# lawmurray/BayesLogit

Measured on NVIDIA B200. Metric: pg_draws_per_sec, higher is better.
Workload: dtype f64

## Files before the change

### bayeslogit_b200/csrc/pg_alt.cuh

```cuda
#pragma once

namespace bl {

template <class Src>
__device__ __forceinline__ double alt_rtinvchi2(Src &s, double h, double trunc)
{
    double h2 = h * h;
    double R = trunc / h2;
    double E1 = s.expon();
    double E2 = s.expon();
    while ((E1 * E1) > (2 * E2 / R)) {
        E1 = s.expon();
        E2 = s.expon();
    }
    double X = 1 + E1 * R;
    X = R / (X * X);
    return h2 * X;
}

__device__ __forceinline__ double alt_pigauss(double x, double z, double lambda)
{
    double sq = sqrt(lambda / x);
    double b = sq * (x * z - 1);
    double a = sq * (x * z + 1) * -1.0;
    return p_norm(b) + ool::exp_(2 * lambda * z) * p_norm(a);
}

enum AltField {
    kAltH = 0,
    kAltTrunc,
    kAltPr,
    kAltCoef,
    kAltLgh,
    kAltLd0, kAltLd1,
    kAltLtB, kAltLtC0, kAltLtLM,
    kAltPrBand,
    kAltSetupDoubles
};
constexpr int kAltStateDoubles = 2 * kAltSetupDoubles;

struct AltState {
    double f[kAltStateDoubles];
    __device__ __forceinline__ double get(int k) const { return f[k]; }
};

struct AltStateRef {
    const double *o;
    size_t stride;
    __device__ __forceinline__ double get(int k) const { return o[(size_t)k * stride]; }
};

__device__ __forceinline__ void alt_plan(double h, int &nfull, int &nrem, double &hrem)
{
    double n = floor((h - 1.0) / 4.0);
    double remain = h - 4.0 * n;
    nfull = (int)n;
    if (remain > 4.0) {
        nrem = 2;
        hrem = 0.5 * remain;
    } else {
        nrem = 1;
        hrem = remain;
    }
}

static __device__ __noinline__ double alt_pr_fp64(double h, double z, double trunc)
{
    const double kLog2 = 0.693147180559945309417232;
    double wl, wr;
    if (z != 0)
        wl = ool::exp_(h * (kLog2 - z)) * alt_pigauss(trunc, z / h, h * h);
    else
        wl = ool::exp_(h * kLog2) * (1.0 - p_gamma_rate(1 / trunc, 0.5, 0.5 * h * h));
    double lambda_z = kPi * kPi * 0.125 + 0.5 * z * z;
    wr = ool::exp_(h * ool::log_((0.5 * kPi) / lambda_z)) * (1.0 - p_gamma_rate(trunc, h, lambda_z));
    return wr / (wr + wl);
}

constexpr double kAltPrBandWidth = 2e-5;

__device__ __forceinline__ float alt_pr_estimate(double h, double z, double trunc)
{
    const float hf = (float)h, zf = (float)z, tf = (float)trunc;
    if (!(zf < 12.0f)) return -1.0f;
    const float s = hf * rsqrtf(tf);
    const float tz = tf * zf / hf;
    const float b = s * (tz - 1.0f), na = s * (tz + 1.0f);
    const float phib = 0.5f * erfcf(-b * 0.70710678f);
    const float wl = exp2f(hf) * (__expf(-hf * zf) * phib
                                  + 0.5f * erfcxf(na * 0.70710678f) * __expf(hf * zf - 0.5f * na * na));
    const float lam = 1.2337005501361697f + 0.5f * zf * zf;
    const float x = tf * lam;
    const float lpre = hf * __logf(x) - x;
    float Q;
    if (x < hf + 1.0f) {
        float term = 1.0f, sum = 1.0f, ap = hf;
        for (int k = 0; k < 60; ++k) {
            ap += 1.0f;
            term *= x / ap;
            sum += term;
            if (term < 1e-8f * sum) break;
        }
        Q = 1.0f - sum * __expf(lpre - lgammaf(hf + 1.0f));
    } else {
        float cf = upper_gamma_cf_f32(hf, x);
        if (!(cf > 0.0f)) return -1.0f;
        Q = cf * __expf(lpre - lgammaf(hf));
    }
    if (!(Q > 0.0f)) return -1.0f;
    const float wr = __expf(hf * __logf(1.5707963267948966f / lam)) * Q;
    const float pr = wr / (wr + wl);
    return pr >= 0.0f && pr <= 1.0f ? pr : -1.0f;
}

template <bool kEstimatePr>
static __device__ __noinline__ void alt_setup(double h, double z, double *out)
{
    const double kLog2 = 0.693147180559945309417232;
    int idx = (int)floor((h - 1.0) * 100.0);
    double trunc = PG_TRUNC_SCHEDULE[idx];
    double rate_z = 0.125 * kPi * kPi + 0.5 * z * z;
    float est = kEstimatePr ? alt_pr_estimate(h, z, trunc) : -1.0f;
    out[kAltH] = h;
    out[kAltTrunc] = trunc;
    out[kAltPr] = est >= 0.0f ? (double)est : alt_pr_fp64(h, z, trunc);
    out[kAltPrBand] = est >= 0.0f ? kAltPrBandWidth : 0.0;
    out[kAltCoef] = ool::exp_(h * kLog2 - 0.5 * 1.8378770664093454835606594728112 );
    out[kAltLgh] = ool::lgamma_(h);
    out[kAltLd0] = ool::log_(h);
    out[kAltLd1] = ool::log_(2.0 + h);
    double b = rate_z * trunc;
    double d1 = b - h;
    double d3 = h - 1.0;
    double c0 = 0.5 * (d1 + sqrt(d1 * d1 + 4.0 * b)) / b;
    out[kAltLtB] = b;
    out[kAltLtC0] = c0;
    out[kAltLtLM] = d3 * ool::log_(d3 / (1.0 - c0)) - d3;
}

template <class St>
__device__ __forceinline__ bool alt_pick_right(double u, const St &st, int o, double z)
{
    const double pr = st.get(o + kAltPr), band = st.get(o + kAltPrBand);
    if (u < pr - band) return true;
    if (u > pr + band || band == 0.0) return false;
    return u < alt_pr_fp64(st.get(o + kAltH), z, st.get(o + kAltTrunc));
}

struct AltLane {
    double X, alpha, sum;
    int trial;
    int phase;
    int nfull;
    int nrem;
    __device__ __forceinline__ void start(int nf, int nr)
    {
        X = 0.0; alpha = 0.0; sum = 0.0; trial = 0; phase = 0; nfull = nf; nrem = nr;
    }
};

__device__ __forceinline__ double alt_coef(double n, double lx3, double ldn, double x, double h,
                                           double coef_h, double &g)
{
    double d_n = 2.0 * n + h;
    if (n != 0)
        g *= (n + h - 1) / n;
    else
        g = 1.0;
    double coef = coef_h * g;
    double log_kernel = -0.5 * (lx3 + d_n * d_n / x) + ldn;
    return coef * ool::exp_(log_kernel);
}

template <class Src, class St>
__device__ __forceinline__ bool alt_pick(Src &src, AltLane &L, double z, const St &st)
{
    const int o = L.nfull > 0 ? 0 : kAltSetupDoubles;
    if (L.trial >= 10000) {
        L.sum += -1.0;
        L.trial = 0;
        if (L.nfull > 0)
            L.nfull--;
        else
            L.nrem--;
        return L.nfull == 0 && L.nrem == 0;
    }
    L.trial++;
    if (alt_pick_right(src.unif(), st, o, z)) {
        L.phase = 1;
    } else {
        L.phase = (st.get(o + kAltH) / z > st.get(o + kAltTrunc)) ? 2 : 3;
        L.alpha = 0.0;
    }
    return false;
}

template <class St>
static __device__ __noinline__ bool alt_series_exact(double X, double u, double h, double trunc, const St &st, int o)
{
    const int max_inner = 200;
    const double coef_h = st.get(o + kAltCoef);
    const double lx3 = ool::log_(X * X * X);
    double g = 1.0;
    double S = alt_coef(0.0, lx3, st.get(o + kAltLd0), X, h, coef_h, g);
    double a_n = S;
    double gt;
    if (X > trunc)
        gt = ool::exp_(h * 0.45158270528945486472619522989488  + (h - 1) * (lx3 * (1.0 / 3.0))
                       - kPi * kPi * 0.125 * X - st.get(o + kAltLgh));
    else
        gt = h * ool::exp_(h * 0.693147180559945309417232 - 0.5 * (1.8378770664093454835606594728112 + lx3)
                           - 0.5 * h * h / X);
    double Y = u * gt;
    int n = 0;
    bool go = true, accept = false;
    while (go && n < max_inner) {
        ++n;
        double prev = a_n;
        double ldn = n == 1 ? st.get(o + kAltLd1) : ool::log_(2.0 * n + h);
        a_n = alt_coef((double)n, lx3, ldn, X, h, coef_h, g);
        bool decreasing = a_n <= prev;
        if (n & 1) {
            S = S - a_n;
            if (Y <= S && decreasing) {
                accept = true;
                go = false;
            }
        } else {
            S = S + a_n;
            if (Y > S && decreasing) go = false;
        }
    }
    return accept;
}

template <class St>
__device__ __forceinline__ bool alt_series_test(double X, double u, double h, double trunc, const St &st, int o)
{
    const double coef_h = st.get(o + kAltCoef);
    const double iX = 1.0 / X;
    const double lx3 = 3.0 * (double)__logf((float)X);
    double lgt;
    if (X > trunc)
        lgt = h * 0.45158270528945486472619522989488 + (h - 1) * (lx3 * (1.0 / 3.0)) - kPi * kPi * 0.125 * X
            - st.get(o + kAltLgh);
    else
        lgt = st.get(o + kAltLd0) + h * 0.693147180559945309417232 - 0.5 * (1.8378770664093454835606594728112 + lx3)
            - 0.5 * h * h * iX;
    const double base = -0.5 * lx3 - lgt;
    const double d0 = h, d1 = h + 2.0, d2 = h + 4.0;
    const double r0 = coef_h * d0 * (double)__expf((float)(base - 0.5 * d0 * d0 * iX));
    const double r1 = coef_h * h * d1 * (double)__expf((float)(base - 0.5 * d1 * d1 * iX));
    const double r2 = coef_h * (0.5 * h * (h + 1.0)) * d2 * (double)__expf((float)(base - 0.5 * d2 * d2 * iX));
    const double band = 1e-5 * (r0 + r1 + r2) + 1e-9;
    const double s1 = r0 - r1;
    if (u <= s1 - band && r1 <= r0 - band) return true;
    const bool not_at_1 = u > s1 + band || r1 > r0 + band;
    if (not_at_1 && u > s1 + r2 + band && r2 <= r1 - band) return false;
    return alt_series_exact(X, u, h, trunc, st, o);
}

template <bool kPickInside = true, class Src, class St>
__device__ __forceinline__ bool alt_trip(Src &src, AltLane &L, double z, const St &st)
{
    if (kPickInside && L.phase == 0) {
        if (alt_pick(src, L, z, st)) return true;
        if (L.phase == 0) return false;
    }
    const int o = L.nfull > 0 ? 0 : kAltSetupDoubles;
    const double h = st.get(o + kAltH);
    const double trunc = st.get(o + kAltTrunc);
    bool chunk_done = false;
    double chunk_val = 0.0;
    if (L.phase == 1) {
        double rate_z = 0.125 * kPi * kPi + 0.5 * z * z;
        if (h == 1.0) {
            L.X = src.expon() / rate_z + trunc;
            L.phase = 4;
        } else {
            double b = st.get(o + kAltLtB), c0 = st.get(o + kAltLtC0);
            double x = b + src.expon() / c0;
            double u = src.unif();
            double l_rho = (h - 1.0) * ool::log_(x) - x * (1.0 - c0);
            if (ool::log_(u) <= l_rho - st.get(o + kAltLtLM)) {
                L.X = trunc * (x / b);
                L.phase = 4;
            }
        }
    } else if (L.phase == 2) {
        if (src.unif() > L.alpha) {
            L.X = alt_rtinvchi2(src, h, trunc);
            L.alpha = ool::exp_(-0.5 * z * z * L.X);
        } else {
            L.phase = 4;
        }
    } else if (L.phase == 3) {
        double X = igauss(src, h / z, h * h);
        if (!(X > trunc)) {
            L.X = X;
            L.phase = 4;
        }
    }
    if (L.phase == 4) {
        const double X = L.X;
        const bool accept = alt_series_test(X, src.unif(), h, trunc, st, o);
        L.phase = 0;
        if (accept) {
            chunk_done = true;
            chunk_val = 0.25 * X;
        }
    }
    if (chunk_done) {
        L.sum += chunk_val;
        L.trial = 0;
        if (L.nfull > 0)
            L.nfull--;
        else
            L.nrem--;
        if (L.nfull == 0 && L.nrem == 0) return true;
    }
    return false;
}

template <class Src>
__device__ double alt_draw(Src &s, double h, double z)
{
    if (h < 1) return 0;
    if (h != h) return h;
    int nfull, nrem;
    double hrem;
    alt_plan(h, nfull, nrem, hrem);
    double zh = fabs(z) * 0.5;
    AltState st;
    if (nfull > 0) alt_setup<false>(4.0, zh, st.f);
    alt_setup<false>(hrem, zh, st.f + kAltSetupDoubles);
    AltLane L;
    L.start(nfull, nrem);
    while (!alt_trip(s, L, zh, st)) {}
    return L.sum;
}

}
```

### bayeslogit_b200/csrc/pg_hybrid.cu

```cuda
#include <algorithm>
#include <cstdlib>
#include <vector>

#include "engine.h"
#include "pg_devroye_fast.cuh"
#include "pg_stream.cuh"

namespace bl {

namespace {

constexpr int kBinThreads = 256;
constexpr int kMetaCounts = 0;
constexpr int kMetaOffsets = 8;
constexpr int kMetaCursor = 16;

__global__ void __launch_bounds__(kBinThreads)
k_hyb_count(const double *__restrict__ h, int n, int *__restrict__ meta)
{
    __shared__ int cnt[8];
    if (threadIdx.x < 8) cnt[threadIdx.x] = 0;
    __syncthreads();
    int local[6] = {0, 0, 0, 0, 0, 0};
    for (int i = blockIdx.x * blockDim.x + threadIdx.x; i < n; i += gridDim.x * blockDim.x)
        local[regime_of(h[i])]++;
#pragma unroll
    for (int r = 0; r < 6; ++r) {
        int v = local[r];
        for (int o = 16; o; o >>= 1) v += __shfl_xor_sync(0xffffffffu, v, o);
        if ((threadIdx.x & 31) == 0 && v) atomicAdd(&cnt[r], v);
    }
    __syncthreads();
    if (threadIdx.x < 6 && cnt[threadIdx.x]) atomicAdd(&meta[kMetaCounts + threadIdx.x], cnt[threadIdx.x]);
}

__global__ void k_hyb_offsets(int *meta)
{
    int acc = 0;
    for (int r = 1; r < 6; ++r) {
        meta[kMetaOffsets + r] = acc;
        meta[kMetaCursor + r] = 0;
        acc += meta[kMetaCounts + r];
    }
}

constexpr int kBinPer = 4;

__global__ void __launch_bounds__(kBinThreads)
k_hyb_scatter(const double *__restrict__ h, int n, int *__restrict__ meta, int *__restrict__ idx,
              double *__restrict__ x)
{
    constexpr int kCells = kBinPer * (kBinThreads / 32);
    __shared__ int wcnt[kCells][8];
    __shared__ int base[8];
    const int lane = threadIdx.x & 31, warp = threadIdx.x >> 5;
    const unsigned lt = (1u << lane) - 1u;
    const int tile_obs = kBinThreads * kBinPer;
    int tiles = (n + tile_obs - 1) / tile_obs;
    for (int tile = blockIdx.x; tile < tiles; tile += gridDim.x) {
        int reg[kBinPer], rank[kBinPer];
#pragma unroll
        for (int k = 0; k < kBinPer; ++k) {
            int i = tile * tile_obs + k * kBinThreads + threadIdx.x;
            reg[k] = i < n ? regime_of(h[i]) : -1;
        }
#pragma unroll
        for (int k = 0; k < kBinPer; ++k) {
            int i = tile * tile_obs + k * kBinThreads + threadIdx.x;
            if (reg[k] == kRegZero) x[i] = 0.0;
            rank[k] = 0;
#pragma unroll
            for (int r = 1; r < 6; ++r) {
                unsigned m = __ballot_sync(0xffffffffu, reg[k] == r);
                if (reg[k] == r) rank[k] = __popc(m & lt);
                if (lane == 0) wcnt[k * (kBinThreads / 32) + warp][r] = __popc(m);
            }
        }
        __syncthreads();
        if (threadIdx.x >= 1 && threadIdx.x < 6) {
            int r = threadIdx.x, run = 0;
            for (int c = 0; c < kCells; ++c) {
                int v = wcnt[c][r];
                wcnt[c][r] = run;
                run += v;
            }
            base[r] = run ? meta[kMetaOffsets + r] + atomicAdd(&meta[kMetaCursor + r], run) : 0;
        }
        __syncthreads();
#pragma unroll
        for (int k = 0; k < kBinPer; ++k) {
            if (reg[k] > 0) {
                int i = tile * tile_obs + k * kBinThreads + threadIdx.x;
                idx[base[reg[k]] + wcnt[k * (kBinThreads / 32) + warp][reg[k]] + rank[k]] = i;
            }
        }
        __syncthreads();
    }
}

template <int R, bool kChains = false>
__global__ void __launch_bounds__(128)
k_hyb_regime(double *__restrict__ x, const double *__restrict__ h, const double *__restrict__ z,
             const int *__restrict__ idx, const int *__restrict__ meta, StreamId id)
{
    const int count = meta[kMetaCounts + R];
    const int *list = idx + meta[kMetaOffsets + R];
    for (int j = blockIdx.x * blockDim.x + threadIdx.x; j < count; j += gridDim.x * blockDim.x) {
        int i = list[j];
        PhiloxSource s;
        if (kChains) open_batch_stream(s, id, i);
        else s.open(id.seed, id.obs0 + (uint64_t)i, id.call_id);
        double b = h[i], zi = z[i], v;
        if (R == kRegNormal) {
            double m = pg_m1(b, zi);
            double var = pg_m2(b, zi) - m * m;
            v = m + sqrt(var) * s.norm();
        } else if (R == kRegSP) {
            sp_draw(s, v, b, zi);
        } else if (R == kRegDevroye) {
            v = devroye_sum_fast(s, (int)b, zi);
        } else if (R == kRegAlt) {
            v = alt_draw(s, b, zi);
        } else {
            v = gamma_sum(s, b, zi, 200);
        }
        x[i] = v;
    }
}

__global__ void __launch_bounds__(128, 8)
k_sp_setup(const double *__restrict__ h, const double *__restrict__ z, const int *__restrict__ idx,
           const int *__restrict__ meta, double *__restrict__ state, int c0, int cap)
{
    const int count = min(meta[kMetaCounts + kRegSP] - c0, cap);
    const int *list = idx + meta[kMetaOffsets + kRegSP] + c0;
    for (int j = blockIdx.x * blockDim.x + threadIdx.x; j < count; j += gridDim.x * blockDim.x) {
        int i = list[j];
        SpState s;
        sp_setup<true>(h[i], z[i], s);
#pragma unroll
        for (int k = 0; k < kSpStateDoubles; ++k) state[(size_t)k * cap + j] = s.f[k];
    }
}

constexpr int kLaneChunk = 128;

constexpr int kRgThreads = 256;

template <int F, int D, int I>
struct RgSlots {
    double f[F][kRgThreads];
    double d[D][kRgThreads];
    uint4 buf[kRgThreads];
    uint32_t blk[kRgThreads];
    int pos[kRgThreads];
    int i[I][kRgThreads];
    int obs[kRgThreads];
    int phase[kRgThreads];
    int perm[kRgThreads];
    int wcnt[kRgThreads / 32][3];
};

struct SpRegroup {
    static constexpr int F = kSpStateDoubles, D = 3, I = 1, kClasses = 2, kRegime = kRegSP;
    using Slots = RgSlots<F, D, I>;
    __device__ static void begin(Slots &S, int t, double shape, double zraw, PhiloxSource &src)
    {
        S.d[0][t] = shape;
        S.d[1][t] = 0.5 * fabs(zraw);
        S.d[2][t] = 2.0;
        S.i[0][t] = 1;
        SpStateRef st{&S.f[0][t], (size_t)kRgThreads};
        S.phase[t] = sp_pick_left(src.unif(), st, shape) ? 1 : 2;
    }
    __device__ static bool advance(Slots &S, int sl, PhiloxSource &src, double &omega)
    {
        SpLane L;
        L.X = S.d[2][sl];
        L.iter = S.i[0][sl];
        L.phase = S.phase[sl];
        const double n = S.d[0][sl];
        SpStateRef st{&S.f[0][sl], (size_t)kRgThreads};
        bool done = sp_trip_staged(src, L, n, S.d[1][sl], st);
        if (!done && L.phase == 0) {
            if (L.iter >= 200) {
                done = true;
            } else {
                L.iter++;
                L.phase = sp_pick_left(src.unif(), st, n) ? 1 : 2;
            }
        }
        if (done) {
            omega = n * 0.25 * L.X;
        } else {
            S.d[2][sl] = L.X;
            S.i[0][sl] = L.iter;
            S.phase[sl] = L.phase;
        }
        return done;
    }
};

struct AltRegroup {
    static constexpr int F = kAltStateDoubles, D = 4, I = 3, kClasses = 3, kRegime = kRegAlt;
    using Slots = RgSlots<F, D, I>;
    __device__ static void load(const Slots &S, int sl, AltLane &L)
    {
        L.X = S.d[1][sl]; L.alpha = S.d[2][sl]; L.sum = S.d[3][sl];
        L.trial = S.i[0][sl]; L.nfull = S.i[1][sl]; L.nrem = S.i[2][sl];
        L.phase = S.phase[sl];
    }
    __device__ static void store(Slots &S, int sl, const AltLane &L)
    {
        S.d[1][sl] = L.X; S.d[2][sl] = L.alpha; S.d[3][sl] = L.sum;
        S.i[0][sl] = L.trial; S.i[1][sl] = L.nfull; S.i[2][sl] = L.nrem;
        S.phase[sl] = L.phase;
    }
    __device__ static void begin(Slots &S, int t, double shape, double zraw, PhiloxSource &src)
    {
        int nfull, nrem;
        double hrem;
        alt_plan(shape, nfull, nrem, hrem);
        AltLane L;
        L.start(nfull, nrem);
        const double zh = 0.5 * fabs(zraw);
        S.d[0][t] = zh;
        AltStateRef st{&S.f[0][t], (size_t)kRgThreads};
        alt_pick(src, L, zh, st);
        store(S, t, L);
    }
    __device__ static bool advance(Slots &S, int sl, PhiloxSource &src, double &omega)
    {
        AltLane L;
        load(S, sl, L);
        const double zh = S.d[0][sl];
        AltStateRef st{&S.f[0][sl], (size_t)kRgThreads};
        bool done = alt_trip<false>(src, L, zh, st);
        while (!done && L.phase == 0) done = alt_pick(src, L, zh, st);
        if (done)
            omega = L.sum;
        else
            store(S, sl, L);
        return done;
    }
};

template <class R, bool kChains = false>
__global__ void __launch_bounds__(kRgThreads)
k_loop_regroup(double *__restrict__ x, const double *__restrict__ h, const double *__restrict__ z,
               const int *__restrict__ idx, const int *__restrict__ meta, const double *__restrict__ state,
               int c0, int cap, StreamId id)
{
    using Slots = typename R::Slots;
    extern __shared__ __align__(16) unsigned char rg_raw[];
    Slots &S = *reinterpret_cast<Slots *>(rg_raw);
    const int count = min(meta[kMetaCounts + R::kRegime] - c0, cap);
    if (count <= 0) return;
    const int *list = idx + meta[kMetaOffsets + R::kRegime] + c0;
    const unsigned full = 0xffffffffu;
    const int t = threadIdx.x, lane = t & 31, warp = t >> 5;
    const unsigned lt_mask = (1u << lane) - 1u;
    constexpr int kWarps = kRgThreads / 32;
    const int gwarp = blockIdx.x * kWarps + warp;
    const int stride = gridDim.x * kWarps * kLaneChunk;
    int cur = gwarp * kLaneChunk, cend = cur + kLaneChunk;

    S.phase[t] = -1;
    __syncthreads();
    for (;;) {
        const bool empty = S.phase[t] < 0;
        const unsigned want = __ballot_sync(full, empty);
        if (want && cur < count) {
            int rank = __popc(want & lt_mask);
            int cand = cur + rank;
            if (cand >= cend) cand += stride - kLaneChunk;
            if (empty && cand < count) {
                const int obs = list[cand];
#pragma unroll
                for (int k = 0; k < R::F; ++k) S.f[k][t] = __ldg(state + (size_t)k * cap + cand);
                S.obs[t] = obs;
                PhiloxSource src;
                if (kChains) open_batch_stream(src, id, obs);
                else src.open(id.seed, id.obs0 + (uint64_t)obs, id.call_id);
                R::begin(S, t, h[obs], z[obs], src);
                S.buf[t] = src.buf;
                S.blk[t] = src.blk;
                S.pos[t] = src.pos;
            }
            cur += __popc(want);
            if (cur >= cend) {
                int over = cur - cend;
                cend += stride;
                cur = cend - kLaneChunk + over;
            }
        }
        const int ph = S.phase[t];
        const unsigned m1 = __ballot_sync(full, ph == 1), m2 = __ballot_sync(full, ph == 2);
        const unsigned m3 = R::kClasses > 2 ? __ballot_sync(full, ph == 3) : 0u;
        if (lane == 0) { S.wcnt[warp][0] = __popc(m1); S.wcnt[warp][1] = __popc(m2); S.wcnt[warp][2] = __popc(m3); }
        __syncthreads();
        int tot1 = 0, tot2 = 0, tot3 = 0, b1 = 0, b2 = 0, b3 = 0;
#pragma unroll
        for (int w = 0; w < kWarps; ++w) {
            int a = S.wcnt[w][0], b = S.wcnt[w][1], c = S.wcnt[w][2];
            if (w < warp) { b1 += a; b2 += b; b3 += c; }
            tot1 += a;
            tot2 += b;
            tot3 += c;
        }
        if (tot1 + tot2 + tot3 == 0) {
            if (!__syncthreads_or(cur < count)) break;
            continue;
        }
        if (ph == 1) S.perm[b1 + __popc(m1 & lt_mask)] = t;
        else if (ph == 3) S.perm[tot1 + b3 + __popc(m3 & lt_mask)] = t;
        else if (ph == 2) S.perm[kRgThreads - 1 - (b2 + __popc(m2 & lt_mask))] = t;
        __syncthreads();
        if (t < tot1 + tot3 || t >= kRgThreads - tot2) {
            const int sl = S.perm[t];
            PhiloxSource src;
            if (kChains) open_batch_stream(src, id, S.obs[sl]);
            else src.open(id.seed, id.obs0 + (uint64_t)S.obs[sl], id.call_id);
            src.buf = S.buf[sl];
            src.blk = S.blk[sl];
            src.pos = S.pos[sl];
            double omega;
            if (R::advance(S, sl, src, omega)) {
                x[S.obs[sl]] = omega;
                S.phase[sl] = -1;
            } else {
                S.buf[sl] = src.buf;
                S.blk[sl] = src.blk;
                S.pos[sl] = src.pos;
            }
        }
        __syncthreads();
    }
}

template <class R, bool kChains>
int regroup_grid()
{
    using Slots = typename R::Slots;
    cudaFuncSetAttribute(k_loop_regroup<R, kChains>, cudaFuncAttributeMaxDynamicSharedMemorySize, (int)sizeof(Slots));
    int per_sm = 0;
    if (cudaOccupancyMaxActiveBlocksPerMultiprocessor(&per_sm, k_loop_regroup<R, kChains>, kRgThreads, sizeof(Slots)) != cudaSuccess || per_sm < 1)
        per_sm = 1;
    int sms = 148, dev = 0;
    if (cudaGetDevice(&dev) == cudaSuccess) cudaDeviceGetAttribute(&sms, cudaDevAttrMultiProcessorCount, dev);
    return sms * per_sm;
}

__global__ void __launch_bounds__(128)
k_alt_setup(const double *__restrict__ h, const double *__restrict__ z, const int *__restrict__ idx,
            const int *__restrict__ meta, double *__restrict__ state, int c0, int cap)
{
    const int count = min(meta[kMetaCounts + kRegAlt] - c0, cap);
    const int *list = idx + meta[kMetaOffsets + kRegAlt] + c0;
    for (int j = blockIdx.x * blockDim.x + threadIdx.x; j < count; j += gridDim.x * blockDim.x) {
        int i = list[j];
        int nfull, nrem;
        double hrem, zh = 0.5 * fabs(z[i]);
        alt_plan(h[i], nfull, nrem, hrem);
        double f[kAltSetupDoubles];
        alt_setup<true>(hrem, zh, f);
#pragma unroll
        for (int k = 0; k < kAltSetupDoubles; ++k) state[(size_t)(kAltSetupDoubles + k) * cap + j] = f[k];
        if (nfull > 0) {
            alt_setup<true>(4.0, zh, f);
#pragma unroll
            for (int k = 0; k < kAltSetupDoubles; ++k) state[(size_t)k * cap + j] = f[k];
        }
    }
}

constexpr int kStateChunk = 1 << 23;
constexpr int kStateDoubles = kSpStateDoubles > kAltStateDoubles ? kSpStateDoubles : kAltStateDoubles;

template <class K>
int resident_grid(K kernel, int threads, int need)
{
    int per_sm = 0;
    if (cudaOccupancyMaxActiveBlocksPerMultiprocessor(&per_sm, kernel, threads, 0) != cudaSuccess || per_sm < 1)
        per_sm = 1;
    int sms = 148;
    int dev = 0;
    if (cudaGetDevice(&dev) == cudaSuccess) cudaDeviceGetAttribute(&sms, cudaDevAttrMultiProcessorCount, dev);
    int cap = sms * per_sm;
    return need < cap ? (need > 0 ? need : 1) : cap;
}

template <int R, bool kChains>
void launch_regime(double *x, const double *h, const double *z, const int *idx, const int *meta,
                   StreamId id, int n, cudaStream_t st)
{
    static const int cap = resident_grid(k_hyb_regime<R, kChains>, 128, 1 << 30);
    int need = (n + 127) / 128;
    k_hyb_regime<R, kChains><<<need < cap ? need : cap, 128, 0, st>>>(x, h, z, idx, meta, id);
    count_launch();
}

}

enum HybStage { kStBin = 0, kStSpSetup, kStSpLoop, kStAltSetup, kStAltLoop, kStGamma, kStNormal, kStDevroye, kStCount };
static bool g_hyb_timing = false;
static std::vector<cudaEvent_t> g_hyb_pool;
struct HybSpan { int stage; int a, b; };
static std::vector<HybSpan> g_hyb_spans;
static int g_hyb_used = 0;

void hybrid_timing_enable(bool on) { g_hyb_timing = on; }

static int hyb_mark(cudaStream_t st)
{
    if ((int)g_hyb_pool.size() <= g_hyb_used) {
        cudaEvent_t e;
        cudaEventCreate(&e);
        g_hyb_pool.push_back(e);
    }
    cudaEventRecord(g_hyb_pool[g_hyb_used], st);
    return g_hyb_used++;
}

struct HybTimer {
    bool on;
    cudaStream_t st;
    int stage, a;
    HybTimer(bool on_, cudaStream_t st_, int stage_) : on(on_), st(st_), stage(stage_), a(on_ ? hyb_mark(st_) : 0) {}
    ~HybTimer() { if (on) g_hyb_spans.push_back(HybSpan{stage, a, hyb_mark(st)}); }
};

int hybrid_timing_last(double *ms8, int *launches8)
{
    if (g_hyb_spans.empty()) return 1;
    for (int k = 0; k < kStCount; ++k) { ms8[k] = 0.0; if (launches8) launches8[k] = 0; }
    if (cudaEventSynchronize(g_hyb_pool[g_hyb_used - 1]) != cudaSuccess) return 1;
    for (const HybSpan &sp : g_hyb_spans) {
        float ms = 0.f;
        cudaEventElapsedTime(&ms, g_hyb_pool[sp.a], g_hyb_pool[sp.b]);
        ms8[sp.stage] += ms;
        if (launches8 && ms > 0.02f) launches8[sp.stage]++;
    }
    return 0;
}

static size_t hybrid_state_offset(int64_t num) { return ((32 + (size_t)num) * sizeof(int) + 15) / 16 * 16; }

size_t hybrid_workspace_bytes(int64_t num)
{
    size_t cap = (size_t)(num < kStateChunk ? num : kStateChunk);
    return hybrid_state_offset(num) + cap * kStateDoubles * sizeof(double);
}

struct SideStream {
    cudaStream_t s = nullptr;
    cudaEvent_t fork = nullptr, join = nullptr;
    cudaStream_t get()
    {
        if (!s) {
            int lo = 0, hi = 0;
            cudaDeviceGetStreamPriorityRange(&lo, &hi);
            cudaStreamCreateWithPriority(&s, cudaStreamNonBlocking, lo);
            cudaEventCreateWithFlags(&fork, cudaEventDisableTiming);
            cudaEventCreateWithFlags(&join, cudaEventDisableTiming);
        }
        return s;
    }
};
static SideStream g_side;

template <bool kChains>
static cudaError_t launch_hybrid_binned_k(double *x, const double *h, const double *z, int num, StreamId id,
                                          void *work, cudaStream_t st)
{
    if (num <= 0) return cudaSuccess;
    int *meta = (int *)work;
    int *idx = meta + 32;
    cudaError_t e = cudaMemsetAsync(meta, 0, 32 * sizeof(int), st);
    if (e != cudaSuccess) return e;
    int tiles = (num + kBinThreads - 1) / kBinThreads;
    int grid = tiles < 148 * 8 ? tiles : 148 * 8;
    int stiles = (num + kBinThreads * kBinPer - 1) / (kBinThreads * kBinPer);
    int sgrid = stiles < 148 * 8 ? stiles : 148 * 8;
    const bool tm = g_hyb_timing;
    if (tm) { g_hyb_spans.clear(); g_hyb_used = 0; }
    {
        HybTimer t(tm, st, kStBin);
        k_hyb_count<<<grid, kBinThreads, 0, st>>>(h, num, meta);
        k_hyb_offsets<<<1, 1, 0, st>>>(meta);
        k_hyb_scatter<<<sgrid, kBinThreads, 0, st>>>(h, num, meta, idx, x);
        count_launch(3);
    }
    static const bool use_side = getenv("BL_HYBRID_NO_SIDE_STREAM") == nullptr;
    cudaStream_t side = use_side ? g_side.get() : st;
    if (use_side) {
        cudaEventRecord(g_side.fork, st);
        cudaStreamWaitEvent(side, g_side.fork, 0);
    }
    {
        HybTimer t(tm, side, kStGamma);
        launch_regime<kRegGamma, kChains>(x, h, z, idx, meta, id, num, side);
    }
    {
        HybTimer t(tm, side, kStNormal);
        launch_regime<kRegNormal, kChains>(x, h, z, idx, meta, id, num, side);
    }
    {
        HybTimer t(tm, side, kStDevroye);
        launch_regime<kRegDevroye, kChains>(x, h, z, idx, meta, id, num, side);
    }
    double *state = (double *)((char *)work + hybrid_state_offset(num));
    const int cap = num < kStateChunk ? num : kStateChunk;
    static const int g_sp_setup = resident_grid(k_sp_setup, 128, 1 << 30);
    static const int g_alt_setup = resident_grid(k_alt_setup, 128, 1 << 30);
    static const int g_sp_regroup = regroup_grid<SpRegroup, kChains>();
    static const int g_alt_regroup = regroup_grid<AltRegroup, kChains>();
    const int rneed = (cap + kLaneChunk * (kRgThreads / 32) - 1) / (kLaneChunk * (kRgThreads / 32));
    const int sneed = (cap + 127) / 128;
    for (int c0 = 0; c0 < num; c0 += cap) {
        {
            HybTimer t(tm, st, kStSpSetup);
            k_sp_setup<<<std::min(sneed, g_sp_setup), 128, 0, st>>>(h, z, idx, meta, state, c0, cap);
        }
        {
            HybTimer t(tm, st, kStSpLoop);
            k_loop_regroup<SpRegroup, kChains><<<std::min(rneed, g_sp_regroup), kRgThreads, sizeof(SpRegroup::Slots), st>>>(x, h, z, idx, meta, state, c0, cap, id);
        }
        count_launch(2);
    }
    for (int c0 = 0; c0 < num; c0 += cap) {
        {
            HybTimer t(tm, st, kStAltSetup);
            k_alt_setup<<<std::min(sneed, g_alt_setup), 128, 0, st>>>(h, z, idx, meta, state, c0, cap);
        }
        {
            HybTimer t(tm, st, kStAltLoop);
            k_loop_regroup<AltRegroup, kChains><<<std::min(rneed, g_alt_regroup), kRgThreads, sizeof(AltRegroup::Slots), st>>>(x, h, z, idx, meta, state, c0, cap, id);
        }
        count_launch(2);
    }
    if (use_side) {
        cudaEventRecord(g_side.join, side);
        cudaStreamWaitEvent(st, g_side.join, 0);
    }
    return cudaGetLastError();
}

cudaError_t launch_hybrid_binned(double *x, const double *h, const double *z, int num, StreamId id,
                                 void *work, cudaStream_t st)
{
    return id.chain_len ? launch_hybrid_binned_k<true>(x, h, z, num, id, work, st)
                        : launch_hybrid_binned_k<false>(x, h, z, num, id, work, st);
}

}
```

### bayeslogit_b200/csrc/pg_samplers.cuh

```cuda
#pragma once

#include "philox.cuh"
#include "specfun.cuh"

#define PG_TABLE_QUAL static __device__ __constant__
#include "pg_tables.h"

namespace bl {

constexpr double kTrunc = 0.64;

namespace ool {
static __device__ __noinline__ double log_(double x) { return ::log(x); }
static __device__ __noinline__ double exp_(double x) { return ::exp(x); }
static __device__ __noinline__ double tan_(double x) { return ::tan(x); }
static __device__ __noinline__ double tanh_(double x) { return ::tanh(x); }
static __device__ __noinline__ double cos_(double x) { return ::cos(x); }
static __device__ __noinline__ double cosh_(double x) { return ::cosh(x); }
static __device__ __noinline__ double atan_(double x) { return ::atan(x); }
static __device__ __noinline__ double lgamma_(double x) { return ::lgamma(x); }
static __device__ __noinline__ double tgamma_(double x) { return ::tgamma(x); }
}


__device__ __forceinline__ double dev_coef(int n, double x)
{
    double K = (n + 0.5) * kPi;
    if (x > kTrunc) return K * exp(-0.5 * K * K * x);
    if (x > 0) {
        double e = -1.5 * (log(0.5 * kPi) + log(x)) + log(K) - 2.0 * (n + 0.5) * (n + 0.5) / x;
        return exp(e);
    }
    return 0.0;
}

__device__ __forceinline__ double dev_right_mass(double Z)
{
    const double t = kTrunc;
    double fz = 0.125 * kPi * kPi + 0.5 * Z * Z;
    double b = sqrt(1.0 / t) * (t * Z - 1);
    double a = sqrt(1.0 / t) * (t * Z + 1) * -1.0;
    double x0 = log(fz) + fz * t;
    double xb = x0 - Z + log_p_norm(b);
    double xa = x0 + Z + log_p_norm(a);
    double qdivp = 4 / kPi * (exp(xb) + exp(xa));
    return 1.0 / (1.0 + qdivp);
}

__device__ __forceinline__ double dev_fz(double Z)
{
    return __dadd_rn(0.125 * kPi * kPi, __dmul_rn(__dmul_rn(0.5, Z), Z));
}

__device__ __forceinline__ double dev_x_right(double E, double fz)
{
    return __dadd_rn(kTrunc, __ddiv_rn(E, fz));
}

__device__ __forceinline__ double dev_x_pair(double E1)
{
    double X = __dadd_rn(1.0, __dmul_rn(E1, kTrunc));
    return __ddiv_rn(kTrunc, __dmul_rn(X, X));
}

__device__ __forceinline__ double dev_x_ig(double N, double mu)
{
    double Y = __dmul_rn(N, N);
    double half_mu = __dmul_rn(0.5, mu);
    double mu_Y = __dmul_rn(mu, Y);
    double rad = __dsqrt_rn(__dadd_rn(__dmul_rn(4.0, mu_Y), __dmul_rn(mu_Y, mu_Y)));
    return __dadd_rn(__dadd_rn(mu, __dmul_rn(half_mu, mu_Y)), -__dmul_rn(half_mu, rad));
}

__device__ __forceinline__ double dev_ig_flip_threshold(double X, double mu)
{
    return __ddiv_rn(mu, __dadd_rn(mu, X));
}

__device__ __forceinline__ double dev_x_ig_flip(double X, double mu)
{
    return __ddiv_rn(__dmul_rn(mu, mu), X);
}

template <class Src>
__device__ __forceinline__ double dev_trunc_igauss(Src &s, double Z)
{
    const double t = kTrunc;
    double X = t + 1.0;
    if (1.0 / kTrunc > Z) {
        double alpha = 0.0;
        while (s.unif() > alpha) {
            double E1 = s.expon();
            double E2 = s.expon();
            while (E1 * E1 > 2 * E2 / t) {
                E1 = s.expon();
                E2 = s.expon();
            }
            X = dev_x_pair(E1);
            alpha = exp(-0.5 * Z * Z * X);
        }
    } else {
        double mu = 1.0 / Z;
        while (X > t) {
            X = dev_x_ig(s.norm(), mu);
            if (s.unif() > dev_ig_flip_threshold(X, mu)) X = dev_x_ig_flip(X, mu);
        }
    }
    return X;
}

template <class Src>
__device__ __forceinline__ double devroye_one(Src &s, double Z, double fz, double right_mass)
{
    for (;;) {
        double X;
        if (s.unif() < right_mass)
            X = dev_x_right(s.expon(), fz);
        else
            X = dev_trunc_igauss(s, Z);
        double S = dev_coef(0, X);
        double Y = s.unif() * S;
        int n = 0;
        for (;;) {
            ++n;
            if (n & 1) {
                S = S - dev_coef(n, X);
                if (Y <= S) return 0.25 * X;
            } else {
                S = S + dev_coef(n, X);
                if (Y > S) break;
            }
        }
    }
}

template <class Src>
__device__ __forceinline__ double devroye_sum(Src &s, int n, double z)
{
    if (n < 1) n = 1;
    double Z = fabs(z) * 0.5;
    double fz = dev_fz(Z);
    double pr = dev_right_mass(Z);
    double sum = 0.0;
    for (int i = 0; i < n; ++i) sum += devroye_one(s, Z, fz, pr);
    return sum;
}


template <class Src>
__device__ __forceinline__ double gamma_sum(Src &s, double b, double z, int T)
{
    if (T < 1) T = 1;
    double x = 0.0;
    double kappa = z * z;
    for (int k = 0; k < T; ++k) {
        double d = (double)k + 0.5;
        double bk = (4 * kPi * kPi) * d * d;
        x += s.gamma(b) / (bk + kappa);
    }
    return 2.0 * x;
}


__device__ __forceinline__ double jj_m1(double b, double z)
{
    z = fabs(z);
    if (z > 1e-12) return b * tanh(z) / z;
    return b * (1 - (1.0 / 3) * pow(z, 2) + (2.0 / 15) * pow(z, 4) - (17.0 / 315) * pow(z, 6));
}

__device__ __forceinline__ double jj_m2(double b, double z)
{
    z = fabs(z);
    if (z > 1e-12) {
        double tz = tanh(z) / z;
        return (b + 1) * b * (tz * tz) + b * ((tanh(z) - z) / (z * z * z));
    }
    double p = 1 - (1.0 / 3) * pow(z, 2) + (2.0 / 15) * pow(z, 4) - (17.0 / 315) * pow(z, 6);
    return (b + 1) * b * (p * p) + b * ((-1.0 / 3) + (2.0 / 15) * pow(z, 2) - (17.0 / 315) * pow(z, 4));
}

__device__ __forceinline__ double pg_m1(double b, double z) { return jj_m1(b, 0.5 * z) * 0.25; }
__device__ __forceinline__ double pg_m2(double b, double z) { return jj_m2(b, 0.5 * z) * 0.0625; }


template <class Src>
__device__ __forceinline__ double igauss(Src &s, double mu, double lambda)
{
    double nu = s.norm();
    double y = nu * nu;
    double x = mu + 0.5 * mu * mu * y / lambda
             - 0.5 * mu / lambda * sqrt(4.0 * mu * lambda * y + (mu * y) * (mu * y));
    if (s.unif() > mu / (mu + x)) x = mu * mu / x;
    return x;
}

template <class Src>
__device__ __noinline__ double ltgamma(Src &s, double shape, double rate, double trunc)
{
    double a = shape;
    double b = rate * trunc;
    if (trunc <= 0.0 || shape < 1.0) return 0.0;
    if (shape == 1.0) return s.expon() / rate + trunc;
    double d1 = b - a;
    double d3 = a - 1.0;
    double c0 = 0.5 * (d1 + sqrt(d1 * d1 + 4.0 * b)) / b;
    double l_M = d3 * ool::log_(d3 / (1.0 - c0)) - d3;
    double x;
    for (;;) {
        x = b + s.expon() / c0;
        double u = s.unif();
        double l_rho = d3 * ool::log_(x) - x * (1.0 - c0);
        if (ool::log_(u) <= l_rho - l_M) break;
    }
    return trunc * (x / b);
}

template <class Src>
__device__ __forceinline__ double tnorm_left(Src &s, double left)
{
    if (left < 0.0) {
        for (;;) {
            double z = s.norm();
            if (z > left) return z;
        }
    }
    double astar = 0.5 * (left + sqrt(left * left + 4.0));
    for (;;) {
        double z = s.expon() / astar + left;
        double rho = ool::exp_(-0.5 * (z - astar) * (z - astar));
        if (s.unif() < rho) return z;
    }
}

template <class Src>
__device__ __forceinline__ double rtinvchi2(Src &s, double scale, double trunc)
{
    double R = trunc / scale;
    double z = tnorm_left(s, 1.0 / sqrt(R));
    return scale / (z * z);
}

}

#include "pg_alt.cuh"
#include "pg_sp.cuh"

namespace bl {


enum Regime { kRegZero = 0, kRegGamma = 1, kRegDevroye = 2, kRegAlt = 3, kRegSP = 4, kRegNormal = 5 };

__device__ __forceinline__ int regime_of(double b)
{
    if (b > 170) return kRegNormal;
    if (b > 13) return kRegSP;
    if (b == 1 || b == 2) return kRegDevroye;
    if (b > 1) return kRegAlt;
    if (b > 0) return kRegGamma;
    return kRegZero;
}

template <class Src>
__device__ double devroye_sum_fast(Src &s, int n, double z);

template <class Src>
__device__ double hybrid_draw(Src &s, double b, double z, int &aux)
{
    aux = 0;
    switch (regime_of(b)) {
    case kRegNormal: {
        double m = pg_m1(b, z);
        double v = pg_m2(b, z) - m * m;
        return m + sqrt(v) * s.norm();
    }
    case kRegSP: {
        double d;
        aux = sp_draw(s, d, b, z);
        return d;
    }
    case kRegDevroye:
        return devroye_sum_fast(s, (int)b, z);
    case kRegAlt:
        return alt_draw(s, b, z);
    case kRegGamma:
        return gamma_sum(s, b, z, 200);
    default:
        return 0.0;
    }
}

}
```

Baseline: 5.080 billion.

## Run alt-regime trips to completion with float-guarded accept tests and deeper series bounds

Adds a staged trip for the alternate PG sampler. Each proposal phase now runs until it produces a candidate and goes straight to the series test, so the per-lane X and alpha no longer need to be stored in the regroup slots. The truncated inverse-chi2 and thinning loops and the left-truncated gamma accept step use lazy exponentials and float logs, with an error band that falls back to exact double evaluation only near the boundary. The series test now evaluates five terms instead of three before falling back to the exact series. The aim is less slot traffic, fewer double-precision transcendentals and fewer exact-series calls, in exchange for more divergence inside the warp and more code complexity.

```diff
diff --git a/bayeslogit_b200/csrc/pg_alt.cuh b/bayeslogit_b200/csrc/pg_alt.cuh
--- a/bayeslogit_b200/csrc/pg_alt.cuh
+++ b/bayeslogit_b200/csrc/pg_alt.cuh
@@ -1,6 +1,13 @@
 #pragma once
 
 namespace bl {
+
+__device__ __forceinline__ double alt_invchi2_x(double E1, double h2, double R)
+{
+    double X = 1 + E1 * R;
+    X = R / (X * X);
+    return h2 * X;
+}
 
 template <class Src>
 __device__ __forceinline__ double alt_rtinvchi2(Src &s, double h, double trunc)
@@ -13,9 +20,7 @@
         E1 = s.expon();
         E2 = s.expon();
     }
-    double X = 1 + E1 * R;
-    X = R / (X * X);
-    return h2 * X;
+    return alt_invchi2_x(E1, h2, R);
 }
 
 __device__ __forceinline__ double alt_pigauss(double x, double z, double lambda)
@@ -248,30 +253,51 @@
         lgt = st.get(o + kAltLd0) + h * 0.693147180559945309417232 - 0.5 * (1.8378770664093454835606594728112 + lx3)
             - 0.5 * h * h * iX;
     const double base = -0.5 * lx3 - lgt;
-    const double d0 = h, d1 = h + 2.0, d2 = h + 4.0;
-    const double r0 = coef_h * d0 * (double)__expf((float)(base - 0.5 * d0 * d0 * iX));
-    const double r1 = coef_h * h * d1 * (double)__expf((float)(base - 0.5 * d1 * d1 * iX));
-    const double r2 = coef_h * (0.5 * h * (h + 1.0)) * d2 * (double)__expf((float)(base - 0.5 * d2 * d2 * iX));
-    const double band = 1e-5 * (r0 + r1 + r2) + 1e-9;
-    const double s1 = r0 - r1;
-    if (u <= s1 - band && r1 <= r0 - band) return true;
-    const bool not_at_1 = u > s1 + band || r1 > r0 + band;
-    if (not_at_1 && u > s1 + r2 + band && r2 <= r1 - band) return false;
+    auto rn = [&](double g, double d) { return coef_h * g * d * (double)__expf((float)(base - 0.5 * d * d * iX)); };
+    const double g2 = 0.5 * h * (h + 1.0), g3 = g2 * (h + 2.0) * (1.0 / 3.0);
+    const double r0 = rn(1.0, h), r1 = rn(h, h + 2.0), r2 = rn(g2, h + 4.0), r3 = rn(g3, h + 6.0),
+                 r4 = rn(g3 * (h + 3.0) * 0.25, h + 8.0);
+    const double band = 1e-5 * (r0 + r1 + r2 + r3 + r4) + 1e-9;
+    auto step = [&](bool odd, double S, double r, double p) {
+        if ((odd ? u <= S - band : u > S + band) && r <= p - band) return 1;
+        return (odd ? u > S + band : u <= S - band) || r > p + band ? 0 : -1;
+    };
+    const double s1 = r0 - r1, s2 = s1 + r2, s3 = s2 - r3;
+    int k = step(true, s1, r1, r0);
+    if (k == 1) return true;
+    if (k == 0) {
+        k = step(false, s2, r2, r1);
+        if (k == 1) return false;
+        if (k == 0) {
+            k = step(true, s3, r3, r2);
+            if (k == 1) return true;
+            if (k == 0 && step(false, s3 + r4, r4, r3) == 1) return false;
+        }
+    }
     return alt_series_exact(X, u, h, trunc, st, o);
 }
 
-template <bool kPickInside = true, class Src, class St>
+__device__ __forceinline__ bool alt_chunk_done(AltLane &L, double X)
+{
+    L.sum += 0.25 * X;
+    L.trial = 0;
+    if (L.nfull > 0)
+        L.nfull--;
+    else
+        L.nrem--;
+    return L.nfull == 0 && L.nrem == 0;
+}
+
+template <class Src, class St>
 __device__ __forceinline__ bool alt_trip(Src &src, AltLane &L, double z, const St &st)
 {
-    if (kPickInside && L.phase == 0) {
+    if (L.phase == 0) {
         if (alt_pick(src, L, z, st)) return true;
         if (L.phase == 0) return false;
     }
     const int o = L.nfull > 0 ? 0 : kAltSetupDoubles;
     const double h = st.get(o + kAltH);
     const double trunc = st.get(o + kAltTrunc);
-    bool chunk_done = false;
-    double chunk_val = 0.0;
     if (L.phase == 1) {
         double rate_z = 0.125 * kPi * kPi + 0.5 * z * z;
         if (h == 1.0) {
@@ -305,21 +331,87 @@
         const double X = L.X;
         const bool accept = alt_series_test(X, src.unif(), h, trunc, st, o);
         L.phase = 0;
-        if (accept) {
-            chunk_done = true;
-            chunk_val = 0.25 * X;
-        }
-    }
-    if (chunk_done) {
-        L.sum += chunk_val;
-        L.trial = 0;
-        if (L.nfull > 0)
-            L.nfull--;
-        else
-            L.nrem--;
-        if (L.nfull == 0 && L.nrem == 0) return true;
+        if (accept) return alt_chunk_done(L, X);
     }
     return false;
+}
+
+static __device__ __noinline__ bool alt_pair_again_exact(uint32_t w1, int k1, uint32_t w2, int k2, double R)
+{
+    const double E1 = philox_expon_ool(w1, k1), E2 = philox_expon_ool(w2, k2);
+    return (E1 * E1) > (2 * E2 / R);
+}
+
+static __device__ __noinline__ bool alt_thin_again_exact(double u, double a)
+{
+    return u > ool::exp_(a);
+}
+
+template <class St>
+__device__ __forceinline__ bool alt_trip_staged(PhiloxSource &src, AltLane &L, double z, const St &st)
+{
+    const int o = L.nfull > 0 ? 0 : kAltSetupDoubles;
+    const double h = st.get(o + kAltH);
+    const double trunc = st.get(o + kAltTrunc);
+    double X;
+    if (L.phase == 1) {
+        if (h == 1.0) {
+            double rate_z = 0.125 * kPi * kPi + 0.5 * z * z;
+            X = src.expon() / rate_z + trunc;
+        } else {
+            const double b = st.get(o + kAltLtB), c0 = st.get(o + kAltLtC0), l_M = st.get(o + kAltLtLM);
+            const double x = b + src.expon() / c0;
+            const double u = src.unif();
+            const float lx = __logf((float)x), lu = __logf((float)u);
+            const double d = (h - 1.0) * (double)lx - x * (1.0 - c0) - l_M - (double)lu;
+            const double band = 1.25e-6 * ((h - 1.0) * (1.0 + fabs((double)lx)) + 2.0 + fabs((double)lu));
+            bool ok;
+            if (!(fabs(d) < 700.0)) ok = sp_ltgamma_accept_exact(u, x, h, c0, l_M);
+            else if (d > band) ok = true;
+            else if (d < -band) ok = false;
+            else ok = sp_ltgamma_accept_exact(u, x, h, c0, l_M);
+            if (!ok) return false;
+            X = trunc * (x / b);
+        }
+    } else if (L.phase == 2) {
+        const double h2 = h * h;
+        const double R = trunc / h2;
+        const double hz2 = -0.5 * z * z;
+        src.word();
+        for (;;) {
+            PhiloxSource::LazyE l1, l2;
+            for (;;) {
+                l1 = src.expon_lazy();
+                l2 = src.expon_lazy();
+                const double e1 = (double)PhiloxSource::approx(l1), e2 = (double)PhiloxSource::approx(l2);
+                const double d = 0.5 * R * (e1 * e1) - e2;
+                const double band = 1.25e-6 * (1.0 + e2 + R * e1 * (1.0 + e1));
+                bool again;
+                if (d > band) again = true;
+                else if (d < -band) again = false;
+                else again = alt_pair_again_exact(l1.w, l1.k, l2.w, l2.k, R);
+                if (!again) break;
+            }
+            X = alt_invchi2_x(philox_expon_ool(l1.w, l1.k), h2, R);
+            const double a = hz2 * X;
+            const double u = src.unif();
+            const float lu = __logf((float)u);
+            const double d = (double)lu - a;
+            const double band = 1.25e-6 * (1.0 + fabs((double)lu));
+            bool again;
+            if (!(a > -700.0)) again = alt_thin_again_exact(u, a);
+            else if (d > band) again = true;
+            else if (d < -band) again = false;
+            else again = alt_thin_again_exact(u, a);
+            if (!again) break;
+        }
+    } else {
+        X = igauss(src, h / z, h * h);
+        if (X > trunc) return false;
+    }
+    const bool accept = alt_series_test(X, src.unif(), h, trunc, st, o);
+    L.phase = 0;
+    return accept && alt_chunk_done(L, X);
 }
 
 template <class Src>
diff --git a/bayeslogit_b200/csrc/pg_hybrid.cu b/bayeslogit_b200/csrc/pg_hybrid.cu
--- a/bayeslogit_b200/csrc/pg_hybrid.cu
+++ b/bayeslogit_b200/csrc/pg_hybrid.cu
@@ -202,17 +202,17 @@
 };
 
 struct AltRegroup {
-    static constexpr int F = kAltStateDoubles, D = 4, I = 3, kClasses = 3, kRegime = kRegAlt;
+    static constexpr int F = kAltStateDoubles, D = 2, I = 3, kClasses = 3, kRegime = kRegAlt;
     using Slots = RgSlots<F, D, I>;
     __device__ static void load(const Slots &S, int sl, AltLane &L)
     {
-        L.X = S.d[1][sl]; L.alpha = S.d[2][sl]; L.sum = S.d[3][sl];
+        L.X = 0.0; L.alpha = 0.0; L.sum = S.d[1][sl];
         L.trial = S.i[0][sl]; L.nfull = S.i[1][sl]; L.nrem = S.i[2][sl];
         L.phase = S.phase[sl];
     }
     __device__ static void store(Slots &S, int sl, const AltLane &L)
     {
-        S.d[1][sl] = L.X; S.d[2][sl] = L.alpha; S.d[3][sl] = L.sum;
+        S.d[1][sl] = L.sum;
         S.i[0][sl] = L.trial; S.i[1][sl] = L.nfull; S.i[2][sl] = L.nrem;
         S.phase[sl] = L.phase;
     }
@@ -235,7 +235,7 @@
         load(S, sl, L);
         const double zh = S.d[0][sl];
         AltStateRef st{&S.f[0][sl], (size_t)kRgThreads};
-        bool done = alt_trip<false>(src, L, zh, st);
+        bool done = alt_trip_staged(src, L, zh, st);
         while (!done && L.phase == 0) done = alt_pick(src, L, zh, st);
         if (done)
             omega = L.sum;
diff --git a/bayeslogit_b200/csrc/pg_samplers.cuh b/bayeslogit_b200/csrc/pg_samplers.cuh
--- a/bayeslogit_b200/csrc/pg_samplers.cuh
+++ b/bayeslogit_b200/csrc/pg_samplers.cuh
@@ -243,8 +243,8 @@
 
 }
 
+#include "pg_sp.cuh"
 #include "pg_alt.cuh"
-#include "pg_sp.cuh"
 
 namespace bl {
 
```

Measured after the change: 5.162 billion (median of 6 runs). 1.02x the previous value.
